# GradientSpaces/LivingScenes

Hardware: AMD Instinct MI355X
Metric: object-instances/sec (encode+match+register), N=1024 pts (higher is better)
Workload: dtype f32 (GEMM products as two-piece f16 splits on the f16 matrix cores, fp32 accumulate: as accurate against fp64 as an fp32 FMA chain)

## Files before the change

### livingscenes_amd/csrc/knn_common.h

```cpp
#pragma once
#include "ls_common.h"

namespace ls {

constexpr int KNN_TQ = 64;
constexpr int KNN_TS = 64;
constexpr int KNN_MAXK = 16;
constexpr int KNN_LD = KNN_TS + 4;

template <bool FMA>
__device__ __forceinline__ float accq(float d, float a, float b) {
#pragma clang fp contract(off)
    const float diff = a - b;
    if constexpr (FMA) {
        return __builtin_fmaf(diff, diff, d);
    } else {
        const float p = diff * diff;
        return d + p;
    }
}

typedef unsigned long long u64;
typedef float f32x2 __attribute__((ext_vector_type(2)));

template <bool FMA>
__device__ __forceinline__ f32x2 accq2(f32x2 d, float q, f32x2 c) {
#pragma clang fp contract(off)
    const f32x2 qq = {q, q};
    const f32x2 diff = qq - c;
    if constexpr (FMA) {
        return __builtin_elementwise_fma(diff, diff, d);
    } else {
        const f32x2 p = diff * diff;
        return d + p;
    }
}

__device__ __forceinline__ u64 make_key(float d, int idx, bool valid) {
    const u64 k = ((u64)__float_as_uint(d) << 32) | (unsigned)idx;
    return valid ? k : ~0ull;
}
__device__ __forceinline__ void key_cx(u64& a, u64& b) {
    const bool sw = b < a;
    const u64 lo = sw ? b : a, hi = sw ? a : b;
    a = lo; b = hi;
}
__device__ __forceinline__ u64 bperm64(int srclane, u64 v) {
    const unsigned lo = (unsigned)__builtin_amdgcn_ds_bpermute(srclane << 2, (int)(unsigned)v);
    const unsigned hi = (unsigned)__builtin_amdgcn_ds_bpermute(srclane << 2, (int)(unsigned)(v >> 32));
    return ((u64)hi << 32) | lo;
}
__device__ __forceinline__ u64 dpp_quad_bcast3(u64 v) {
    const unsigned lo = (unsigned)__builtin_amdgcn_update_dpp(0, (int)(unsigned)v, 0xFF, 0xF, 0xF, true);
    const unsigned hi = (unsigned)__builtin_amdgcn_update_dpp(0, (int)(unsigned)(v >> 32), 0xFF, 0xF, 0xF, true);
    return ((u64)hi << 32) | lo;
}
__device__ __forceinline__ u64 dpp_row_shr1(u64 v) {
    const unsigned lo = (unsigned)__builtin_amdgcn_update_dpp(0, (int)(unsigned)v, 0x111, 0xF, 0xF, false);
    const unsigned hi = (unsigned)__builtin_amdgcn_update_dpp(0, (int)(unsigned)(v >> 32), 0x111, 0xF, 0xF, false);
    return ((u64)hi << 32) | lo;
}

template <int CC>
struct Stager {
    static constexpr int U2 = CC / 16;
    static constexpr int PER = 3 * U2;
    float4 r[PER];
    __device__ __forceinline__ void load(const float* __restrict__ base, const int* rowmap, int row0, int nrows, size_t row_f,
                                         int C, int c0, int tid) {
        const int rr = tid >> 2, q = tid & 3;
        const int gr = rowmap ? rowmap[rr] : ((row0 + rr) < nrows ? row0 + rr : -1);
        const float* p = base + (size_t)(gr >= 0 ? gr : 0) * row_f + c0 + q * 4;
#pragma unroll
        for (int u = 0; u < PER; ++u) {
            const float4 v = *reinterpret_cast<const float4*>(p + (size_t)(u / U2) * C + (u % U2) * 16);
            r[u] = gr >= 0 ? v : make_float4(0.f, 0.f, 0.f, 0.f);
        }
    }
    __device__ __forceinline__ void store_pairs(float* lds, int PR, int tid) const {
        const int rr = tid >> 2, q = tid & 3;
        float* p0 = lds + (rr >> 1) * PR + (rr & 1) + 2 * (q * 12);
#pragma unroll
        for (int u = 0; u < PER; ++u) {
            float* p = p0 + 2 * ((u % U2) * 48 + (u / U2));
            p[0] = r[u].x; p[6] = r[u].y; p[12] = r[u].z; p[18] = r[u].w;
        }
    }
    __device__ __forceinline__ void store(float* lds, int ROW, int tid) const {
        const int rr = tid >> 2, q = tid & 3;
        float* p0 = lds + rr * ROW + q * 12;
#pragma unroll
        for (int u = 0; u < PER; ++u) {
            float* p = p0 + (u % U2) * 48 + (u / U2);
            p[0] = r[u].x; p[3] = r[u].y; p[6] = r[u].z; p[9] = r[u].w;
        }
    }
};


template <bool DEDUP>
__device__ __forceinline__ void merge_keys(u64 k0, u64 k1, u64 k2, u64 k3, u64& lkg, u64& kk, int K, int lane) {
    const int e16 = lane & 15, rowbase = lane & 48;
    u64 m64 = __ballot(k0 < kk);
    while (m64) {
        const unsigned rb = (unsigned)(m64 >> rowbase) & 0xFFFFu;
        bool rowhas = rb != 0;
        const int srclane = rowbase + __builtin_ctz(rb | 0x10000u);
        const u64 cand = bperm64(srclane, k0);
        const bool is_src = lane == srclane;
        k0 = is_src ? k1 : k0; k1 = is_src ? k2 : k1; k2 = is_src ? k3 : k2; k3 = is_src ? ~0ull : k3;
        if constexpr (DEDUP) {
            const u64 d64 = __ballot(rowhas & (lkg == cand));
            rowhas = rowhas & (((unsigned)(d64 >> rowbase) & 0xFFFFu) == 0u);
        }
        const u64 l64 = __ballot(rowhas & (lkg < cand));
        const int pos = __builtin_popcount((unsigned)(l64 >> rowbase) & 0xFFFFu);
        const u64 up = dpp_row_shr1(lkg);
        const bool s1 = rowhas & (e16 == pos), s2 = rowhas & (e16 > pos);
        lkg = s1 ? cand : (s2 ? up : lkg);
        kk = bperm64(rowbase + K - 1, lkg);
        m64 = __ballot(k0 < kk);
    }
}

template <bool DEDUP>
__device__ __forceinline__ void select_tile(const float* ldist, u64 (&lk)[4], u64 (&rkey)[4], int s0, int Ns, int K, int wave,
                                            int lane) {
    const int e16 = lane & 15;
#pragma unroll
    for (int g = 0; g < 4; ++g) {
        const int qrow = wave * 16 + g * 4 + (lane >> 4);
        const float4 dv = *reinterpret_cast<const float4*>(&ldist[qrow * KNN_LD + e16 * 4]);
        const int cbase = s0 + e16;
        u64 k0 = make_key(dv.x, cbase, cbase < Ns), k1 = make_key(dv.y, cbase + 16, cbase + 16 < Ns);
        u64 k2 = make_key(dv.z, cbase + 32, cbase + 32 < Ns), k3 = make_key(dv.w, cbase + 48, cbase + 48 < Ns);
        key_cx(k0, k1); key_cx(k2, k3); key_cx(k0, k2); key_cx(k1, k3); key_cx(k1, k2);
        merge_keys<DEDUP>(k0, k1, k2, k3, lk[g], rkey[g], K, lane);
    }
}

__device__ __forceinline__ void seed_lists(const u64* lseed, u64 (&lk)[4], u64 (&rkey)[4], int K, int wave, int lane) {
#pragma unroll
    for (int g = 0; g < 4; ++g) {
        const int qrow = wave * 16 + g * 4 + (lane >> 4);
        merge_keys<true>(lseed[qrow * 16 + (lane & 15)], ~0ull, ~0ull, ~0ull, lk[g], rkey[g], K, lane);
    }
}

template <bool FMA>
__device__ __forceinline__ float row_distance(const float* __restrict__ a, const float* __restrict__ b, int C) {
    float d = 0.0f;
    for (int c4 = 0; c4 < C; c4 += 4) {
        const float4 ax = *reinterpret_cast<const float4*>(a + c4), ay = *reinterpret_cast<const float4*>(a + C + c4),
                     az = *reinterpret_cast<const float4*>(a + 2 * C + c4);
        const float4 bx = *reinterpret_cast<const float4*>(b + c4), by = *reinterpret_cast<const float4*>(b + C + c4),
                     bz = *reinterpret_cast<const float4*>(b + 2 * C + c4);
        d = accq<FMA>(d, ax.x, bx.x); d = accq<FMA>(d, ay.x, by.x); d = accq<FMA>(d, az.x, bz.x);
        d = accq<FMA>(d, ax.y, bx.y); d = accq<FMA>(d, ay.y, by.y); d = accq<FMA>(d, az.y, bz.y);
        d = accq<FMA>(d, ax.z, bx.z); d = accq<FMA>(d, ay.z, by.z); d = accq<FMA>(d, az.z, bz.z);
        d = accq<FMA>(d, ax.w, bx.w); d = accq<FMA>(d, ay.w, by.w); d = accq<FMA>(d, az.w, bz.w);
    }
    return d;
}

template <bool FMA>
__device__ __forceinline__ void compute_seed_keys(u64* lseed, const int32_t* __restrict__ seed_idx, int seed_n, bool seed_by_row,
                                                  const float* __restrict__ dbase, const float* __restrict__ sbase, const int* lqrow,
                                                  int b, int q0, int Ns, int C, int tid) {
    const size_t row_f = (size_t)3 * C;
#pragma unroll
    for (int u = 0; u < 4; ++u) {
        const int p = tid + u * 256;
        const int q = p >> 4, e = p & 15;
        const int r = lqrow[q];
        int sidx = -1;
        if (r >= 0) sidx = seed_idx[((size_t)b * seed_n + (seed_by_row ? r : q0 + q)) * 16 + e];
        u64 key = ~0ull;
        if (sidx >= 0 && sidx < Ns) key = make_key(row_distance<FMA>(dbase + (size_t)r * row_f, sbase + (size_t)sidx * row_f, C), sidx, true);
        lseed[q * 16 + e] = key;
    }
}

__device__ __forceinline__ void write_lists(const u64 (&lk)[4], int b, int q0, int Nd, int K, int wave, int lane, int splits, int sp,
                                            u64* __restrict__ partial, int32_t* __restrict__ idx_out, float* __restrict__ dist_out) {
#pragma unroll
    for (int g = 0; g < 4; ++g) {
        const int q = q0 + wave * 16 + g * 4 + (lane >> 4);
        const int e = lane & 15;
        if (q < Nd && splits > 1) {
            partial[(((size_t)b * Nd + q) * splits + sp) * 16 + e] = e < K ? lk[g] : ~0ull;
        } else if (q < Nd && e < K) {
            const size_t o = ((size_t)b * Nd + q) * K + e;
            const unsigned hi = (unsigned)(lk[g] >> 32), lo = (unsigned)lk[g];
            idx_out[o] = hi == 0xFFFFFFFFu ? -1 : (int)lo;
            if (dist_out) dist_out[o] = hi == 0xFFFFFFFFu ? INFINITY : __uint_as_float(hi);
        }
    }
}

template <int CTRL>
__device__ __forceinline__ unsigned dpp_mov(unsigned v) {
    return (unsigned)__builtin_amdgcn_update_dpp(0, (int)v, CTRL, 0xF, 0xF, true);
}
template <int M>
__device__ __forceinline__ unsigned lane_xor(unsigned v, int lane) {
    if constexpr (M == 1) return dpp_mov<0xB1>(v);
    else if constexpr (M == 2) return dpp_mov<0x4E>(v);
    else if constexpr (M == 3) return dpp_mov<0x1B>(v);
    else if constexpr (M == 7) return dpp_mov<0x141>(v);
    else if constexpr (M == 15) return dpp_mov<0x140>(v);
    else if constexpr (M < 32) return (unsigned)__builtin_amdgcn_ds_swizzle((int)v, (M << 10) | 0x1F);
    else return (unsigned)__builtin_amdgcn_ds_bpermute((lane ^ M) << 2, (int)v);
}
template <int M>
__device__ __forceinline__ constexpr int pair_bit() { return (M & (M + 1)) == 0 ? (M + 1) / 2 : M; }

template <int M>
__device__ __forceinline__ void cx32(unsigned& v, int lane) {
    const unsigned o = lane_xor<M>(v, lane);
    v = (lane & pair_bit<M>()) == 0 ? min(v, o) : max(v, o);
}
template <int M>
__device__ __forceinline__ void cx64(u64& v, int lane) {
    const u64 o = ((u64)lane_xor<M>((unsigned)(v >> 32), lane) << 32) | lane_xor<M>((unsigned)v, lane);
    const bool lt = o < v, takemin = (lane & pair_bit<M>()) == 0;
    v = (takemin == lt) ? o : v;
}
__device__ __forceinline__ unsigned kth_smallest_upper_bound(unsigned v, int K) {
    unsigned ans = 0;
#pragma unroll
    for (int bit = 30; bit >= 15; --bit) {
        const unsigned t = ans | ((1u << bit) - 1u);
        const int cnt = __builtin_popcountll(__ballot(v <= t));
        ans |= cnt >= K ? 0u : (1u << bit);
    }
    return min(ans | 0x7FFFu, 0x7F800000u);
}

#define LS_SORT16(CX, v, lane)                                                                                         \
    CX<1>(v, lane);                                                                                                    \
    CX<3>(v, lane); CX<1>(v, lane);                                                                                    \
    CX<7>(v, lane); CX<2>(v, lane); CX<1>(v, lane);                                                                    \
    CX<15>(v, lane); CX<4>(v, lane); CX<2>(v, lane); CX<1>(v, lane);

#define LS_SORT32(CX, v, lane)                                                                                         \
    LS_SORT16(CX, v, lane)                                                                                             \
    CX<31>(v, lane); CX<8>(v, lane); CX<4>(v, lane); CX<2>(v, lane); CX<1>(v, lane);

#define LS_SORT64(CX, v, lane)                                                                                         \
    CX<1>(v, lane);                                                                                                    \
    CX<3>(v, lane); CX<1>(v, lane);                                                                                    \
    CX<7>(v, lane); CX<2>(v, lane); CX<1>(v, lane);                                                                    \
    CX<15>(v, lane); CX<4>(v, lane); CX<2>(v, lane); CX<1>(v, lane);                                                   \
    CX<31>(v, lane); CX<8>(v, lane); CX<4>(v, lane); CX<2>(v, lane); CX<1>(v, lane);                                   \
    CX<63>(v, lane); CX<16>(v, lane); CX<8>(v, lane); CX<4>(v, lane); CX<2>(v, lane); CX<1>(v, lane);


}
```

### livingscenes_amd/csrc/knn_mfma.hip

```cpp
#include "knn_common.h"

namespace ls {

typedef float f32x16 __attribute__((ext_vector_type(16)));


template <int CC>
struct QuadRow {
    float4 v[6];
    __device__ __forceinline__ void load(const float* __restrict__ row, int lane, int round = 0) {
        const int off = round * 32 + (lane & 3) * 8;
#pragma unroll
        for (int x = 0; x < 3; ++x)
#pragma unroll
            for (int h = 0; h < 2; ++h) v[x * 2 + h] = *reinterpret_cast<const float4*>(row + x * CC + off + 4 * h);
    }
};
template <int CC, bool FMA, bool LAST>
__device__ __forceinline__ float quad_round(float d, const QuadRow<CC>& q, const QuadRow<CC>& c) {
#pragma clang fp contract(off)
    float t[24];
#pragma unroll
    for (int h = 0; h < 2; ++h)
#pragma unroll
        for (int x = 0; x < 3; ++x) {
            const float4 a = q.v[x * 2 + h], b = c.v[x * 2 + h];
            const float d0 = a.x - b.x, d1 = a.y - b.y, d2 = a.z - b.z, d3 = a.w - b.w;
            t[(h * 4 + 0) * 3 + x] = FMA ? d0 : d0 * d0;
            t[(h * 4 + 1) * 3 + x] = FMA ? d1 : d1 * d1;
            t[(h * 4 + 2) * 3 + x] = FMA ? d2 : d2 * d2;
            t[(h * 4 + 3) * 3 + x] = FMA ? d3 : d3 * d3;
        }
#pragma unroll
    for (int s = 0; s < 4; ++s) {
#pragma unroll
        for (int j = 0; j < 24; ++j) d = FMA ? __builtin_fmaf(t[j], t[j], d) : d + t[j];
        if (s < 3)
            d = __int_as_float(__builtin_amdgcn_update_dpp(0, __float_as_int(d), 0x90, 0xF, 0xF, false));
        else if (!LAST)
            d = __int_as_float(__builtin_amdgcn_update_dpp(0, __float_as_int(d), 0x93, 0xF, 0xF, false));
    }
    return d;
}
template <int CC, bool FMA>
__device__ __forceinline__ float quad_pair_distance(const QuadRow<CC>& q0, const float* __restrict__ qrow, const float* __restrict__ crow,
                                                    int lane) {
    QuadRow<CC> c;
    c.load(crow, lane, 0);
    if constexpr (CC == 32) {
        return quad_round<CC, FMA, true>(0.0f, q0, c);
    } else {
        float d = quad_round<CC, FMA, false>(0.0f, q0, c);
#pragma unroll
        for (int r = 1; r < CC / 32; ++r) {
            QuadRow<CC> q;
            q.load(qrow, lane, r);
            c.load(crow, lane, r);
            d = (r == CC / 32 - 1) ? quad_round<CC, FMA, true>(d, q, c) : quad_round<CC, FMA, false>(d, q, c);
        }
        return d;
    }
}

typedef _Float16 f16x8k __attribute__((ext_vector_type(8)));
typedef _Float16 kh2_t __attribute__((ext_vector_type(2)));
typedef float kf2_t __attribute__((ext_vector_type(2)));
constexpr int KNN_CENTRE_ROWS = 16;
template <int KK, int WPT>
__global__ __launch_bounds__(64 * WPT) void knn_prep_f16_tile_kernel(const float* __restrict__ f, const float* __restrict__ fc, int Nc, int N, int Npad,
                                                                    unsigned short* __restrict__ out, float* __restrict__ norms, float* __restrict__ iscale,
                                                                    int32_t* __restrict__ zero_buf, long long zero_n) {
    constexpr int D = KK * 16, KPW = KK / WPT, DW = KPW * 16;
    static_assert(KK % WPT == 0 && DW <= 64, "a wave's dims fit one lane each for the centre");
    __shared__ __attribute__((aligned(16))) float lmu[WPT][64];
    __shared__ float lamax[WPT][32], lsum[WPT][32];
    for (long long i = (long long)blockIdx.x * (64 * WPT) + threadIdx.x; i < zero_n; i += (long long)gridDim.x * (64 * WPT)) zero_buf[i] = 0;
    const int lane = threadIdx.x & 63, w = __builtin_amdgcn_readfirstlane(threadIdx.x >> 6), j = lane & 31, h = lane >> 5;
    const int tpi = Npad >> 5, b = blockIdx.x / tpi, tile = blockIdx.x % tpi, r = tile * 32 + j;
    const bool live = r < N;
    const float* rp = f + ((size_t)b * N + (live ? r : 0)) * D + w * DW + h * 8;
    float4 x[KPW][2];
#pragma unroll
    for (int kk = 0; kk < KPW; ++kk) { x[kk][0] = *reinterpret_cast<const float4*>(rp + kk * 16); x[kk][1] = *reinterpret_cast<const float4*>(rp + kk * 16 + 4); }
    {
        const int nc = min(Nc, KNN_CENTRE_ROWS);
        const float* cp = fc + (size_t)b * Nc * D + w * DW + lane;
        if (lane < DW) {
            float s0 = 0.f, s1 = 0.f, s2 = 0.f, s3 = 0.f;
            for (int rr = 0; rr + 3 < nc; rr += 4) {
                s0 += cp[(size_t)rr * D]; s1 += cp[(size_t)(rr + 1) * D]; s2 += cp[(size_t)(rr + 2) * D]; s3 += cp[(size_t)(rr + 3) * D];
            }
            for (int rr = nc & ~3; rr < nc; ++rr) s0 += cp[(size_t)rr * D];
            lmu[w][lane] = ((s0 + s1) + (s2 + s3)) / (float)nc;
        }
        __builtin_amdgcn_s_waitcnt(0xc07f);
        __builtin_amdgcn_wave_barrier();
    }
    float c[KPW][8];
    float amax = 0.f;
#pragma unroll
    for (int kk = 0; kk < KPW; ++kk) {
        const float4 m0 = *reinterpret_cast<const float4*>(&lmu[w][kk * 16 + h * 8]), m1 = *reinterpret_cast<const float4*>(&lmu[w][kk * 16 + h * 8 + 4]);
        const float4 x0 = x[kk][0], x1 = x[kk][1];
        const float t[8] = {x0.x - m0.x, x0.y - m0.y, x0.z - m0.z, x0.w - m0.w, x1.x - m1.x, x1.y - m1.y, x1.z - m1.z, x1.w - m1.w};
#pragma unroll
        for (int i = 0; i < 8; ++i) { c[kk][i] = live ? t[i] : 0.f; amax = fmaxf(amax, fabsf(t[i])); }
    }
    amax = fmaxf(amax, __shfl_xor(amax, 32, 64));
    if (h == 0) lamax[w][j] = amax;
    __syncthreads();
#pragma unroll
    for (int u = 0; u < WPT; ++u) amax = fmaxf(amax, lamax[u][j]);
    unsigned be = (__float_as_uint(amax) >> 23) & 0xffu;
    be = be < 15u ? 15u : be;
    const float sc = live ? __uint_as_float((268u - be) << 23) : 0.f;
    unsigned short* op = out + ((((size_t)b * tpi + tile) * KK + w * KPW) * 64 + lane) * 8;
    float s = 0.f;
#pragma unroll
    for (int kk = 0; kk < KPW; ++kk) {
        unsigned pk[4];
#pragma unroll
        for (int i = 0; i < 4; ++i) {
            const float c0 = c[kk][2 * i], c1 = c[kk][2 * i + 1];
            s += c0 * c0 + c1 * c1;
            const kh2_t hv = __builtin_convertvector(kf2_t{c0 * sc, c1 * sc}, kh2_t);
            pk[i] = __builtin_bit_cast(unsigned, hv);
        }
        uint4 wv;
        wv.x = pk[0]; wv.y = pk[1]; wv.z = pk[2]; wv.w = pk[3];
        *reinterpret_cast<uint4*>(op + (size_t)kk * 512) = wv;
    }
    s += __shfl_xor(s, 32, 64);
    if (h == 0) lsum[w][j] = s;
    __syncthreads();
    if (w == 0 && h == 0 && live) {
        float t = lsum[0][j];
#pragma unroll
        for (int u = 1; u < WPT; ++u) t += lsum[u][j];
        norms[(size_t)b * N + r] = t;
        iscale[(size_t)b * N + r] = __uint_as_float((be - 14u) << 23);
    }
}
#ifndef LS_KF_PK
#define LS_KF_PK 1
#endif
constexpr int KF_QT = 32;
constexpr int KF_WAVES = 8;
constexpr int KF_LCAP = 64;
constexpr int KF_MAXNS = KF_WAVES * 4 * 32;

template <int CC>
struct KfLds {
    float qrows[KF_QT][3 * CC];
    float qnx[KF_QT], qny[KF_QT];
    unsigned hm[KF_QT][64];
    float T[KF_QT];
    int cnt[KF_QT];
    int base[KF_QT + 1];
    unsigned short list[KF_QT][KF_LCAP];
    unsigned plist[KF_QT * KF_LCAP];
    u64 keys[KF_QT][KF_LCAP];
};

template <int CC, bool FMA>
__device__ __noinline__ u64 kf_brute_row(const float* __restrict__ qrow, const float* __restrict__ sbase, int Ns, int lane) {
    constexpr int RF = 3 * CC;
    const int quad = lane >> 2;
    const bool qlast = (lane & 3) == 3;
    QuadRow<CC> qv;
    qv.load(qrow, lane);
    u64 best = ~0ull;
    for (int base = 0; base < Ns; base += 48) {
        u64 ks[3];
#pragma unroll
        for (int u = 0; u < 3; ++u) {
            const int c = base + u * 16 + quad;
            const bool v = c < Ns;
            ks[u] = make_key(quad_pair_distance<CC, FMA>(qv, qrow, sbase + (size_t)(v ? c : 0) * RF, lane), c, v & qlast);
        }
        const int src = ((lane & 15) << 2) + 3;
        const u64 n0 = bperm64(src, ks[0]), n1 = bperm64(src, ks[1]), n2 = bperm64(src, ks[2]);
        u64 k = lane < 16 ? best : (lane < 32 ? n0 : (lane < 48 ? n1 : n2));
        LS_SORT64(cx64, k, lane)
        best = k;
    }
    return best;
}

template <int CC, bool FMA, int TPW>
__global__ __launch_bounds__(64 * KF_WAVES, FMA ? 3 : 4) void knn_fused_kernel(const float* __restrict__ dstf, const float* __restrict__ srcf, const int32_t* __restrict__ dst_rows,
                                                                  const unsigned short* __restrict__ dq, const unsigned short* __restrict__ sq,
                                                                  const float* __restrict__ nrm_dst, const float* __restrict__ nrm_src,
                                                                  const float* __restrict__ isc_dst, const float* __restrict__ isc_src, int Nd, int dst_n,
                                                                  int dst_npad, int Ns, int ns_pad, int K, int qtiles, float eps,
                                                                  int32_t* __restrict__ idx_out, float* __restrict__ dist_out, int32_t* __restrict__ surv_cnt) {
    constexpr int D = 3 * CC, KK = D / 16, RF = 3 * CC;
    __shared__ __attribute__((aligned(16))) KfLds<CC> L;
    const int tid = threadIdx.x, lane = tid & 63;
    const int wave = __builtin_amdgcn_readfirstlane(tid >> 6);
    const int l31 = lane & 31, lh = lane >> 5;
    const int logical = xcd_remap(blockIdx.x, gridDim.x);
    const int b = logical / qtiles, q0 = (logical - b * qtiles) * KF_QT;
    const unsigned short* dqb = dq + (size_t)b * dst_npad * D;
    const unsigned short* sqb = sq + (size_t)b * ns_pad * D;
    const float* sbase = srcf + (size_t)b * Ns * RF;
    const float* dbase = dstf + (size_t)b * dst_n * RF;
    const int ntiles = ns_pad >> 5;

    for (int i = tid; i < KF_QT * (RF / 4); i += 64 * KF_WAVES) {
        const int qr = i / (RF / 4), c4 = i - qr * (RF / 4);
        const int q = min(q0 + qr, Nd - 1);
        const int r = dst_rows ? dst_rows[(size_t)b * Nd + q] : q;
        *reinterpret_cast<float4*>(&L.qrows[qr][c4 * 4]) = *reinterpret_cast<const float4*>(dbase + (size_t)r * RF + c4 * 4);
    }
    if (tid < KF_QT) {
        const int q = q0 + tid;
        const int r = q < Nd ? (dst_rows ? dst_rows[(size_t)b * Nd + q] : q) : 0;
        const float nq = nrm_dst[(size_t)b * dst_n + r], iq = isc_dst[(size_t)b * dst_n + r];
        L.qnx[tid] = q < Nd ? nq : 0.f;
        L.qny[tid] = q < Nd ? -2.0f * iq : 0.f;
        L.cnt[tid] = 0;
    }
    for (int i = tid; i < KF_QT * 64; i += 64 * KF_WAVES) (&L.hm[0][0])[i] = 0x7F800000u;

    f16x8k a[KK];
    {
        const int qi = q0 + l31;
        const int r = qi < Nd ? (dst_rows ? dst_rows[(size_t)b * Nd + qi] : qi) : 0;
        const unsigned short* ap = dqb + ((size_t)(r >> 5) * KK * 64 + lh * 32 + (r & 31)) * 8;
#pragma unroll
        for (int kk = 0; kk < KK; ++kk) a[kk] = __builtin_bit_cast(f16x8k, *reinterpret_cast<const uint4*>(ap + (size_t)kk * 512));
    }
    f32x16 S[TPW];
    float cns[TPW], cic[TPW];
    {
        f16x8k bf[2][KK];
        auto load_b = [&](int t, f16x8k (&dstb)[KK]) {
            const int tg = min(wave + KF_WAVES * t, ntiles - 1);
            const unsigned short* bp = sqb + ((size_t)tg * KK * 64 + lane) * 8;
#pragma unroll
            for (int kk = 0; kk < KK; ++kk) dstb[kk] = __builtin_bit_cast(f16x8k, *reinterpret_cast<const uint4*>(bp + (size_t)kk * 512));
        };
        load_b(0, bf[0]);
#pragma unroll
        for (int t = 0; t < TPW; ++t) {
            if (t + 1 < TPW) load_b(t + 1, bf[(t + 1) & 1]);
            const int cg = min((wave + KF_WAVES * t) * 32 + l31, Ns - 1);
            cns[t] = nrm_src[(size_t)b * Ns + cg];
            cic[t] = isc_src[(size_t)b * Ns + cg];
#pragma unroll
            for (int r = 0; r < 16; ++r) S[t][r] = 0.0f;
#pragma unroll
            for (int kk = 0; kk < KK; ++kk) S[t] = __builtin_amdgcn_mfma_f32_32x32x16_f16(a[kk], bf[t & 1][kk], S[t], 0, 0, 0);
        }
    }
    __syncthreads();
    bool colv[TPW];
#pragma unroll
    for (int t = 0; t < TPW; ++t) colv[t] = (wave + KF_WAVES * t) < ntiles && (wave + KF_WAVES * t) * 32 + l31 < Ns;
#if LS_KF_PK
    {
        const int slot = (wave & 1) * 32 + l31;
        kf2_t cn2[TPW], ci2[TPW];
#pragma unroll
        for (int t = 0; t < TPW; ++t) { const float cn = colv[t] ? cns[t] : INFINITY; cn2[t] = kf2_t{cn, cn}; ci2[t] = kf2_t{cic[t], cic[t]}; }
        const kf2_t eps2 = {eps, eps};
#pragma unroll
        for (int r = 0; r < 16; r += 2) {
            const int qr = (r & 3) + 8 * (r >> 2) + 4 * lh;
            const kf2_t qx = *reinterpret_cast<const kf2_t*>(&L.qnx[qr]), qy = *reinterpret_cast<const kf2_t*>(&L.qny[qr]);
            float hm0 = INFINITY, hm1 = INFINITY;
#pragma unroll
            for (int t = 0; t < TPW; ++t) {
                const kf2_t nn = qx + cn2[t], w = qy * ci2[t];
                const kf2_t sv = {S[t][r], S[t][r + 1]};
                const kf2_t dh = __builtin_elementwise_fma(sv, w, nn), e = eps2 * nn;
                const kf2_t hi = dh + e;
                kf2_t lo = dh - e;
                hm0 = fminf(hm0, hi.x); hm1 = fminf(hm1, hi.y);
                asm volatile("" : "+v"(lo));
                S[t][r] = lo.x; S[t][r + 1] = lo.y;
            }
            const float h0 = fmaxf(hm0, 0.0f), h1 = fmaxf(hm1, 0.0f);
            if (h0 < INFINITY) atomicMin(&L.hm[qr][slot], __float_as_uint(h0));
            if (h1 < INFINITY) atomicMin(&L.hm[qr + 1][slot], __float_as_uint(h1));
            if ((r & 3) == 2) __builtin_amdgcn_sched_barrier(0);
        }
    }
#else
    {
        const int slot = (wave & 1) * 32 + l31;
#pragma unroll
        for (int r = 0; r < 16; ++r) {
            const int qr = (r & 3) + 8 * (r >> 2) + 4 * lh;
            const float2 qn = make_float2(L.qnx[qr], L.qny[qr]);
            float hmin = INFINITY;
#pragma unroll
            for (int t = 0; t < TPW; ++t) {
                const float nn = qn.x + cns[t], w = qn.y * cic[t];
                const float dh = __builtin_fmaf(S[t][r], w, nn), e = eps * nn;
                hmin = colv[t] ? fminf(hmin, dh + e) : hmin;
                float lo = dh - e;
                asm volatile("" : "+v"(lo));
                S[t][r] = lo;
            }
            const float h = fmaxf(hmin, 0.0f);
            if (h < INFINITY) atomicMin(&L.hm[qr][slot], __float_as_uint(h));
            if ((r & 3) == 3) __builtin_amdgcn_sched_barrier(0);
        }
    }
#endif
    __syncthreads();
#pragma unroll
    for (int u = 0; u < KF_QT / KF_WAVES; ++u) {
        const int qr = wave * (KF_QT / KF_WAVES) + u;
        const unsigned tb = kth_smallest_upper_bound(L.hm[qr][lane], K < 64 ? K : 64);
        if (lane == 0) L.T[qr] = __uint_as_float(tb);
    }
    __syncthreads();
    {
        unsigned mask[TPW];
#pragma unroll
        for (int t = 0; t < TPW; ++t) mask[t] = 0;
#pragma unroll
        for (int r = 0; r < 16; ++r) {
            const float Tr = L.T[(r & 3) + 8 * (r >> 2) + 4 * lh];
#pragma unroll
            for (int t = 0; t < TPW; ++t) mask[t] |= (S[t][r] > Tr) ? 0u : (1u << r);
        }
#pragma unroll
        for (int t = 0; t < TPW; ++t) {
            const int cg = (wave + KF_WAVES * t) * 32 + l31;
            unsigned m = colv[t] ? mask[t] : 0u;
            while (m) {
                const int r = __builtin_ctz(m);
                m &= m - 1;
                const int qr = (r & 3) + 8 * (r >> 2) + 4 * lh;
                if (q0 + qr < Nd) {
                    const int pos = atomicAdd(&L.cnt[qr], 1);
                    if (pos < KF_LCAP) L.list[qr][pos] = (unsigned short)cg;
                }
            }
        }
    }
    __syncthreads();
    if (wave == 0) {
        const int c = (lane < KF_QT && L.cnt[lane] <= KF_LCAP) ? L.cnt[lane] : 0;
        int incl = c;
#pragma unroll
        for (int o = 1; o < KF_QT; o <<= 1) {
            const int v = __shfl_up(incl, o, 64);
            incl += lane >= o ? v : 0;
        }
        if (lane < KF_QT) L.base[lane] = incl - c;
        if (lane == KF_QT - 1) L.base[KF_QT] = incl;
        if (lane < KF_QT && q0 + lane < Nd && surv_cnt) surv_cnt[(size_t)b * Nd + q0 + lane] = -(L.cnt[lane] > KF_LCAP ? Ns : L.cnt[lane]) - 1;
    }
    __syncthreads();
    for (int i = tid; i < KF_QT * KF_LCAP; i += 64 * KF_WAVES) {
        const int qr = i / KF_LCAP, j = i - qr * KF_LCAP;
        const int c = L.cnt[qr];
        if (c <= KF_LCAP && j < c) L.plist[L.base[qr] + j] = (unsigned)L.list[qr][j] | ((unsigned)qr << 16) | ((unsigned)j << 21);
    }
    __syncthreads();
    {
        const int P = L.base[KF_QT];
        const int Q = wave * 16 + (lane >> 2);
        const bool qlast = (lane & 3) == 3;
        struct Pair { unsigned ent; bool v; QuadRow<CC> c; };
        auto fetch = [&](int p0, Pair& pr) {
            const int p = p0 + Q;
            pr.v = p < P;
            pr.ent = L.plist[pr.v ? p : 0];
            pr.c.load(sbase + (size_t)(pr.ent & 0xFFFFu) * RF, lane, 0);
        };
        auto finish = [&](const Pair& pr) {
            const int cand = pr.ent & 0xFFFFu, qr = (pr.ent >> 16) & 31, slot = pr.ent >> 21;
            const float* qrow = &L.qrows[qr][0];
            QuadRow<CC> qv;
            qv.load(qrow, lane);
            float d;
            if constexpr (CC == 32) {
                d = quad_round<CC, FMA, true>(0.0f, qv, pr.c);
            } else {
                const float* crow = sbase + (size_t)cand * RF;
                d = quad_round<CC, FMA, false>(0.0f, qv, pr.c);
#pragma unroll
                for (int r = 1; r < CC / 32; ++r) {
                    QuadRow<CC> q, c;
                    q.load(qrow, lane, r);
                    c.load(crow, lane, r);
                    d = (r == CC / 32 - 1) ? quad_round<CC, FMA, true>(d, q, c) : quad_round<CC, FMA, false>(d, q, c);
                }
            }
            if (pr.v && qlast) L.keys[qr][slot] = make_key(d, cand, true);
        };
        if (P > 0) {
            Pair pa, pb;
            fetch(0, pa);
            for (int p0 = 0; p0 < P; p0 += 2 * 16 * KF_WAVES) {
                fetch(p0 + 16 * KF_WAVES, pb);
                __builtin_amdgcn_sched_barrier(0);
                finish(pa);
                if (p0 + 16 * KF_WAVES < P) {
                    fetch(p0 + 2 * 16 * KF_WAVES, pa);
                    __builtin_amdgcn_sched_barrier(0);
                    finish(pb);
                }
            }
        }
    }
    __syncthreads();
    auto emit = [&](int qr, u64 k, int e) {
        const int q = q0 + qr;
        if (q < Nd && e < K) {
            const size_t o = ((size_t)b * Nd + q) * K + e;
            const unsigned hi = (unsigned)(k >> 32), lw = (unsigned)k;
            idx_out[o] = hi == 0xFFFFFFFFu ? -1 : (int)lw;
            if (dist_out) dist_out[o] = hi == 0xFFFFFFFFu ? INFINITY : __uint_as_float(hi);
        }
    };
#pragma unroll
    for (int u = 0; u < KF_QT / KF_WAVES; u += 2) {
        const int qa = wave * (KF_QT / KF_WAVES) + u, qb = qa + 1;
        const int ca = L.cnt[qa], cb = L.cnt[qb];
        if (ca <= 32 && cb <= 32) {
            const int qr = lh ? qb : qa, c = lh ? cb : ca;
            u64 k = l31 < c ? L.keys[qr][l31] : ~0ull;
            LS_SORT32(cx64, k, lane)
            emit(qr, k, l31);
        } else {
#pragma unroll
            for (int h = 0; h < 2; ++h) {
                const int qr = h ? qb : qa, c = h ? cb : ca;
                u64 k;
                if (c <= KF_LCAP) {
                    k = lane < c ? L.keys[qr][lane] : ~0ull;
                    LS_SORT64(cx64, k, lane)
                } else {
                    k = q0 + qr < Nd ? kf_brute_row<CC, FMA>(&L.qrows[qr][0], sbase, Ns, lane) : ~0ull;
                }
                emit(qr, k, lane);
            }
        }
    }
}

static inline size_t pad32(size_t n) { return (n + 31) & ~(size_t)31; }
static int knn_prep_launch(const float* f, const float* fc, int Nc, int B, int N, int Npad, int D, unsigned short* out, float* norms, float* iscale, hipStream_t st) {
    const int tiles = B * (Npad / 32);
    if (D == 96)
        hipLaunchKernelGGL((knn_prep_f16_tile_kernel<6, 3>), dim3(tiles), dim3(192), 0, st, f, fc, Nc, N, Npad, out, norms, iscale, (int32_t*)nullptr, 0LL);
    else
        hipLaunchKernelGGL((knn_prep_f16_tile_kernel<12, 4>), dim3(tiles), dim3(256), 0, st, f, fc, Nc, N, Npad, out, norms, iscale, (int32_t*)nullptr, 0LL);
    LS_LAUNCH_CHECK();
    return LS_OK;
}
int knn_sweep_max_ns() { return KF_MAXNS; }

struct KfScratch { float *nsrc, *ndst, *isrc, *idst; int32_t* cnt; unsigned short *sq, *dq; size_t bytes; };
static KfScratch kf_layout(void* scratch, int B, int Nd, int dst_n, int Ns, int D, bool self) {
    char* sc = (char*)scratch;
    size_t off = 0;
    auto take = [&](size_t bytes) { char* p = sc + off; off = (off + bytes + 255) & ~(size_t)255; return p; };
    KfScratch k;
    k.cnt = (int32_t*)take((size_t)B * Nd * sizeof(int32_t));
    k.nsrc = (float*)take((size_t)B * Ns * sizeof(float));
    k.ndst = self ? k.nsrc : (float*)take((size_t)B * dst_n * sizeof(float));
    k.isrc = (float*)take((size_t)B * Ns * sizeof(float));
    k.idst = self ? k.isrc : (float*)take((size_t)B * dst_n * sizeof(float));
    k.sq = (unsigned short*)take((size_t)B * pad32(Ns) * D * sizeof(unsigned short));
    k.dq = self ? k.sq : (unsigned short*)take((size_t)B * pad32(dst_n) * D * sizeof(unsigned short));
    k.bytes = off;
    return k;
}
size_t knn_sweep_scratch_bytes(int B, int Nd, int dst_n, int Ns, int C) { return kf_layout(nullptr, B, Nd, dst_n, Ns, 3 * C, false).bytes; }

template <int CC>
static int knn_sweep_launch_t(const float* dst, const float* src, const int32_t* dst_rows, int B, int Nd, int dst_n, int Ns, int K, bool fma,
                              int32_t* idx_out, float* dist_out, void* scratch, hipStream_t st) {
    constexpr int D = 3 * CC;
    const KfScratch k = kf_layout(scratch, B, Nd, dst_n, Ns, D, dst == src);
    const int ns_pad = (int)pad32(Ns), dst_npad = (int)pad32(dst_n);
    int rc = knn_prep_launch(src, src, Ns, B, Ns, ns_pad, D, k.sq, k.nsrc, k.isrc, st);
    if (rc != LS_OK) return rc;
    if (dst != src) {
        rc = knn_prep_launch(dst, src, Ns, B, dst_n, dst_npad, D, k.dq, k.ndst, k.idst, st);
        if (rc != LS_OK) return rc;
    }
    const int qtiles = cdiv(Nd, KF_QT), tpw = cdiv(ns_pad / 32, KF_WAVES);
    const float epsF = 1.02f * 0.0009765625f + 6.0f * (float)(D + 4) * 5.9604645e-8f + 9.5367431640625e-7f + 4.76837158203125e-7f;
#define LS_KF(T) do { if (fma) hipLaunchKernelGGL((knn_fused_kernel<CC, true, T>), dim3(B * qtiles), dim3(64 * KF_WAVES), 0, st, dst, src, dst_rows, k.dq, k.sq, k.ndst, k.nsrc, k.idst, k.isrc, Nd, dst_n, dst_npad, Ns, ns_pad, K, qtiles, epsF, idx_out, dist_out, k.cnt); \
                   else hipLaunchKernelGGL((knn_fused_kernel<CC, false, T>), dim3(B * qtiles), dim3(64 * KF_WAVES), 0, st, dst, src, dst_rows, k.dq, k.sq, k.ndst, k.nsrc, k.idst, k.isrc, Nd, dst_n, dst_npad, Ns, ns_pad, K, qtiles, epsF, idx_out, dist_out, k.cnt); } while (0)
    if (tpw <= 1) LS_KF(1); else if (tpw == 2) LS_KF(2); else LS_KF(4);
#undef LS_KF
    LS_LAUNCH_CHECK();
    return LS_OK;
}

int knn_sweep_launch(const float* dst, const float* src, const int32_t* dst_rows, int B, int Nd, int dst_n, int Ns, int C, int K,
                     bool fma, int32_t* idx_out, float* dist_out, const int32_t* , int , int , void* scratch,
                     hipStream_t st) {
    LS_REQUIRE(C == 32 || C == 64, "knn_sweep: only C == 32 / 64 layers are supported (C=%d)", C);
    LS_REQUIRE((int)pad32(Ns) <= KF_MAXNS && K <= KNN_MAXK, "knn_sweep: Ns=%d K=%d beyond the fused kernel (Ns <= %d, K <= 16)", Ns, K, KF_MAXNS);
    if (C == 32) return knn_sweep_launch_t<32>(dst, src, dst_rows, B, Nd, dst_n, Ns, K, fma, idx_out, dist_out, scratch, st);
    return knn_sweep_launch_t<64>(dst, src, dst_rows, B, Nd, dst_n, Ns, K, fma, idx_out, dist_out, scratch, st);
}

__global__ __launch_bounds__(256) void knn_stats_kernel(const int32_t* __restrict__ surv_cnt, long long nq, unsigned long long* __restrict__ out) {
    unsigned long long s = 0;
    for (long long i = (long long)blockIdx.x * 256 + threadIdx.x; i < nq; i += (long long)gridDim.x * 256) {
        const int c = surv_cnt[i];
        s += (unsigned long long)(c < 0 ? -(c + 1) : 0);
    }
    for (int o = 32; o > 0; o >>= 1) s += __shfl_xor(s, o, 64);
    if ((threadIdx.x & 63) == 0) atomicAdd(&out[0], s);
    if (blockIdx.x == 0 && threadIdx.x == 0) atomicAdd(&out[1], (unsigned long long)nq);
}
int knn_sweep_stats_launch(const void* scratch, int B, int Nd, int dst_n, int Ns, unsigned long long* out, hipStream_t st) {
    const size_t nq = (size_t)B * Nd;
    (void)dst_n; (void)Ns;
    hipLaunchKernelGGL(knn_stats_kernel, dim3((unsigned)std::min<size_t>(cdiv((long long)nq, 256), 256)), dim3(256), 0, st, (const int32_t*)scratch, (long long)nq, out);
    LS_LAUNCH_CHECK();
    return LS_OK;
}

}
```

### livingscenes_amd/csrc/knn_xyz.hip

```cpp
#include "knn_common.h"

namespace ls {

constexpr int KX_CH = 1024;

template <bool FMA, bool SINGLE>
__global__ __launch_bounds__(256, 4) void knn_xyz_kernel(const float* __restrict__ dst, const float* __restrict__ src,
                                                      const int32_t* __restrict__ dst_rows, int Nd, int dst_n, int Ns, int K,
                                                      int32_t* __restrict__ idx_out, float* __restrict__ dist_out, int qpw,
                                                      int qblocks) {
    __shared__ u64 lsurv[4][KX_CH + 1];
    const int lane = threadIdx.x & 63;
    const int wave = __builtin_amdgcn_readfirstlane(threadIdx.x >> 6);
    const int logical = xcd_remap(blockIdx.x, gridDim.x);
    const int b = logical / qblocks, qb = logical % qblocks;
    const float* sb = src + (size_t)b * Ns * 3;
    const float* db = dst + (size_t)b * dst_n * 3;
    u64* ls = lsurv[wave];
    constexpr bool single = SINGLE;

    f32x2 cx[8], cy[8], cz[8];
    auto load_chunk = [&](int c0) {
#pragma unroll
        for (int j = 0; j < 8; ++j) {
            const int ca = c0 + lane + 64 * j, cb = ca + 512;
            const int la = min(ca, Ns - 1), lb = min(cb, Ns - 1);
            const float ax = sb[(size_t)la * 3 + 0], ay = sb[(size_t)la * 3 + 1], az = sb[(size_t)la * 3 + 2];
            const float bx = sb[(size_t)lb * 3 + 0], by = sb[(size_t)lb * 3 + 1], bz = sb[(size_t)lb * 3 + 2];
            cx[j] = f32x2{ca < Ns ? ax : INFINITY, cb < Ns ? bx : INFINITY};
            cy[j] = f32x2{ca < Ns ? ay : INFINITY, cb < Ns ? by : INFINITY};
            cz[j] = f32x2{ca < Ns ? az : INFINITY, cb < Ns ? bz : INFINITY};
        }
    };
    if (single) load_chunk(0);

    const int qbase = (qb * 4 + wave) * qpw;
    for (int qi = 0; qi < qpw; ++qi) {
        const int q = qbase + qi;
        if (q >= Nd) break;
        const int r = __builtin_amdgcn_readfirstlane(dst_rows ? dst_rows[(size_t)b * Nd + q] : q);
        const float qx = db[(size_t)r * 3 + 0], qy = db[(size_t)r * 3 + 1], qz = db[(size_t)r * 3 + 2];
        u64 best = ~0ull;
        for (int c0 = 0; c0 < Ns; c0 += KX_CH) {
            if (!single) load_chunk(c0);
            f32x2 d[8];
            unsigned mn = 0x7F800000u;
#pragma unroll
            for (int j = 0; j < 8; ++j) {
                f32x2 a = accq2<FMA>(f32x2{0.0f, 0.0f}, qx, cx[j]);
                a = accq2<FMA>(a, qy, cy[j]);
                a = accq2<FMA>(a, qz, cz[j]);
                d[j] = a;
                mn = min(mn, min(__float_as_uint(a.x), __float_as_uint(a.y)));
            }
            unsigned thr = kth_smallest_upper_bound(mn, K);
            thr = min(thr, (unsigned)__builtin_amdgcn_readlane((int)(unsigned)(best >> 32), K - 1));
            thr = min(thr, 0x7F7FFFFFu);
            int n = 0;
#pragma unroll
            for (int jj = 0; jj < 16; ++jj) {
                const int j = jj & 7;
                const float dv = jj < 8 ? d[j].x : d[j].y;
                const int c = c0 + lane + 64 * j + (jj < 8 ? 0 : 512);
                const bool pass = __float_as_uint(dv) <= thr;
                const u64 bal = __ballot(pass);
                const int pos = n + (int)__builtin_amdgcn_mbcnt_hi((unsigned)(bal >> 32), __builtin_amdgcn_mbcnt_lo((unsigned)bal, 0u));
                ls[pass ? pos : KX_CH] = make_key(dv, c, true);
                n += __builtin_popcountll(bal);
            }
            __builtin_amdgcn_wave_barrier();
            int pos = 0;
            if (c0 == 0) {
                u64 k = lane < n ? ls[lane] : ~0ull;
                if (n <= 32) { LS_SORT32(cx64, k, lane) }
                else { LS_SORT64(cx64, k, lane) }
                best = k;
                pos = 64;
            }
            for (; pos < n; pos += 48) {
                u64 k = best;
                if (lane >= 16) {
                    const int i = pos + lane - 16;
                    k = i < n ? ls[i] : ~0ull;
                }
                LS_SORT64(cx64, k, lane)
                best = k;
            }
            __builtin_amdgcn_wave_barrier();
        }
        if (lane < K) {
            const size_t o = ((size_t)b * Nd + q) * K + lane;
            const unsigned hi = (unsigned)(best >> 32), lo = (unsigned)best;
            idx_out[o] = hi == 0xFFFFFFFFu ? -1 : (int)lo;
            if (dist_out) dist_out[o] = hi == 0xFFFFFFFFu ? INFINITY : __uint_as_float(hi);
        }
    }
}

int knn_xyz_launch(const float* dst, const float* src, const int32_t* dst_rows, int B, int Nd, int dst_n, int Ns, int K, bool fma,
                   int32_t* idx_out, float* dist_out, hipStream_t st) {
    int qpw = 16;
    while (qpw > 1 && (long long)B * cdiv(Nd, 4 * qpw) < 1024) qpw >>= 1;
    const int qblocks = cdiv(Nd, 4 * qpw);
    const bool single = Ns <= KX_CH;
#define LS_KX(F, S) hipLaunchKernelGGL((knn_xyz_kernel<F, S>), dim3(B * qblocks), dim3(256), 0, st, dst, src, dst_rows, Nd, dst_n, Ns, K, \
                                       idx_out, dist_out, qpw, qblocks)
    if (fma) { if (single) LS_KX(true, true); else LS_KX(true, false); }
    else { if (single) LS_KX(false, true); else LS_KX(false, false); }
#undef LS_KX
    LS_LAUNCH_CHECK();
    return LS_OK;
}


__device__ __forceinline__ int cdiv_dev(int a, int b) { return (a + b - 1) / b; }
constexpr int KSM_Q = 8, KSM_S = 32, KSM_CCH = 128;
constexpr int KSM_ROW = 3 * KSM_CCH + 4;

template <bool FMA>
__global__ __launch_bounds__(256, 2) void knn_small_kernel(const float* __restrict__ dstf, const float* __restrict__ srcf,
                                                           const int32_t* __restrict__ dst_rows, int Nd, int dst_n, int Ns, int C, int K,
                                                           int32_t* __restrict__ idx_out, float* __restrict__ dist_out, int qblocks) {
    LS_LATENCY_CRITICAL();
    __shared__ __attribute__((aligned(16))) float lq[KSM_Q * KSM_ROW];
    __shared__ __attribute__((aligned(16))) float lc[KSM_S * KSM_ROW];
    __shared__ float ldist[KSM_Q][KSM_S + 1];
    __shared__ int lqrow[KSM_Q];
    const int tid = threadIdx.x, lane = tid & 63, wave = tid >> 6;
    const int logical = xcd_remap(blockIdx.x, gridDim.x);
    const int b = logical / qblocks, q0 = (logical % qblocks) * KSM_Q;
    const size_t row_f = (size_t)3 * C;
    const float* dbase = dstf + (size_t)b * dst_n * row_f;
    const float* sbase = srcf + (size_t)b * Ns * row_f;
    if (tid < KSM_Q) {
        const int q = q0 + tid;
        lqrow[tid] = q < Nd ? (dst_rows ? dst_rows[(size_t)b * Nd + q] : q) : -1;
    }
    __syncthreads();
    const int qi = tid >> 5, ci = tid & 31;
    u64 lk = ~0ull, rkey = ~0ull;
    const int nch = cdiv_dev(C, KSM_CCH);
    const int sr = tid >> 3, sc = (tid & 7) * 4;
#define KSM_PF_LIST(F) F(0, 0) F(0, 1) F(0, 2) F(0, 3) F(1, 0) F(1, 1) F(1, 2) F(1, 3) F(2, 0) F(2, 1) F(2, 2) F(2, 3)
#define KSM_PF_DECL(x, m) float4 pf_##x##_##m;
#define KSM_PF_LOAD(x, m) pf_##x##_##m = *reinterpret_cast<const float4*>(rp + (size_t)x * C + min(m * 32, cwp - 32));
#define KSM_PF_STORE(x, m) \
    if (sc + m * 32 < cw) *reinterpret_cast<float4*>(&lc[sr * KSM_ROW + x * KSM_CCH + sc + m * 32]) = pf_##x##_##m;
    KSM_PF_LIST(KSM_PF_DECL)
#define KSM_PREFETCH(S0, CH)                                                                                  \
    {                                                                                                         \
        const int c0p = (CH) * KSM_CCH, cwp = min(C - c0p, KSM_CCH);                                          \
        const float* rp = sbase + (size_t)min((S0) + sr, Ns - 1) * row_f + c0p + sc;                          \
        KSM_PF_LIST(KSM_PF_LOAD)        \
    }
    KSM_PREFETCH(0, 0)
    for (int s0 = 0; s0 < Ns; s0 += KSM_S) {
        float d = 0.0f;
        for (int ch = 0; ch < nch; ++ch) {
            const int c0 = ch * KSM_CCH, cw = min(C - c0, KSM_CCH);
            __syncthreads();
            if (nch > 1 || s0 == 0) {
                const int gr = lqrow[qi];
                for (int x = 0; x < 3; ++x)
                    for (int c4 = ci * 4; c4 < cw; c4 += 128)
                        *reinterpret_cast<float4*>(&lq[qi * KSM_ROW + x * KSM_CCH + c4]) =
                            gr >= 0 ? *reinterpret_cast<const float4*>(dbase + (size_t)gr * row_f + (size_t)x * C + c0 + c4)
                                    : make_float4(0.f, 0.f, 0.f, 0.f);
            }
            KSM_PF_LIST(KSM_PF_STORE)
            __syncthreads();
            {
                int nch2 = ch + 1, ns0 = s0;
                if (nch2 == nch) { nch2 = 0; ns0 = s0 + KSM_S; }
                KSM_PREFETCH(min(ns0, Ns - 1), nch2)
            }
            const float* qp = &lq[qi * KSM_ROW];
            const float* cp = &lc[ci * KSM_ROW];
#pragma unroll 2
            for (int c4 = 0; c4 < cw; c4 += 4) {
                const float4 ax = *reinterpret_cast<const float4*>(qp + c4), ay = *reinterpret_cast<const float4*>(qp + KSM_CCH + c4),
                             az = *reinterpret_cast<const float4*>(qp + 2 * KSM_CCH + c4);
                const float4 bx = *reinterpret_cast<const float4*>(cp + c4), by = *reinterpret_cast<const float4*>(cp + KSM_CCH + c4),
                             bz = *reinterpret_cast<const float4*>(cp + 2 * KSM_CCH + c4);
                d = accq<FMA>(d, ax.x, bx.x); d = accq<FMA>(d, ay.x, by.x); d = accq<FMA>(d, az.x, bz.x);
                d = accq<FMA>(d, ax.y, bx.y); d = accq<FMA>(d, ay.y, by.y); d = accq<FMA>(d, az.y, bz.y);
                d = accq<FMA>(d, ax.z, bx.z); d = accq<FMA>(d, ay.z, by.z); d = accq<FMA>(d, az.z, bz.z);
                d = accq<FMA>(d, ax.w, bx.w); d = accq<FMA>(d, ay.w, by.w); d = accq<FMA>(d, az.w, bz.w);
            }
        }
        ldist[qi][ci] = d;
        __syncthreads();
        if (wave < 2) {
            const int qr = wave * 4 + (lane >> 4), e = lane & 15;
            const int ca = s0 + e, cb = s0 + e + 16;
            const bool live = lqrow[qr] >= 0;
            u64 k0 = make_key(ldist[qr][e], ca, live && ca < Ns), k1 = make_key(ldist[qr][e + 16], cb, live && cb < Ns);
            key_cx(k0, k1);
            merge_keys<false>(k0, k1, ~0ull, ~0ull, lk, rkey, K, lane);
        }
    }
    if (wave < 2) {
        const int qr = wave * 4 + (lane >> 4), e = lane & 15, q = q0 + qr;
        if (q < Nd && e < K) {
            const size_t o = ((size_t)b * Nd + q) * K + e;
            const unsigned hi = (unsigned)(lk >> 32), lo = (unsigned)lk;
            idx_out[o] = hi == 0xFFFFFFFFu ? -1 : (int)lo;
            if (dist_out) dist_out[o] = hi == 0xFFFFFFFFu ? INFINITY : __uint_as_float(hi);
        }
    }
}

int knn_small_launch(const float* dst, const float* src, const int32_t* dst_rows, int B, int Nd, int dst_n, int Ns, int C, int K, bool fma,
                     int32_t* idx_out, float* dist_out, hipStream_t st) {
    LS_REQUIRE(C % 4 == 0, "knn_small: C=%d must be a multiple of 4", C);
    const int qblocks = cdiv(Nd, KSM_Q);
    if (fma)
        hipLaunchKernelGGL(knn_small_kernel<true>, dim3(B * qblocks), dim3(256), 0, st, dst, src, dst_rows, Nd, dst_n, Ns, C, K, idx_out,
                           dist_out, qblocks);
    else
        hipLaunchKernelGGL(knn_small_kernel<false>, dim3(B * qblocks), dim3(256), 0, st, dst, src, dst_rows, Nd, dst_n, Ns, C, K, idx_out,
                           dist_out, qblocks);
    LS_LAUNCH_CHECK();
    return LS_OK;
}

}
```

Before: 57110.

## Compact KNN survivor lists with wave scans and overlap query staging with MFMA

The fused KNN filter kernel now builds its flat survivor pair list directly. A per-wave DPP inclusive scan and one atomic per wave replace the per-query list, the block-wide prefix pass and two extra barriers. Slot assignment into the per-query key buffers moves into the refine fetch step. Query-row staging into LDS is deferred until after the MFMA distance products, so its global loads can overlap the matrix work. The xyz kernel skips stores when a ballot is empty, and its launch heuristic targets more blocks. This adds a flood fallback when the shared pair list overflows, and registers rise from holding staged rows.

```diff
diff --git a/livingscenes_amd/csrc/knn_common.h b/livingscenes_amd/csrc/knn_common.h
--- a/livingscenes_amd/csrc/knn_common.h
+++ b/livingscenes_amd/csrc/knn_common.h
@@ -59,6 +59,16 @@
     const unsigned lo = (unsigned)__builtin_amdgcn_update_dpp(0, (int)(unsigned)v, 0x111, 0xF, 0xF, false);
     const unsigned hi = (unsigned)__builtin_amdgcn_update_dpp(0, (int)(unsigned)(v >> 32), 0x111, 0xF, 0xF, false);
     return ((u64)hi << 32) | lo;
+}
+
+__device__ __forceinline__ int wave_incl_scan(int v) {
+    v += __builtin_amdgcn_update_dpp(0, v, 0x111, 0xF, 0xF, false);
+    v += __builtin_amdgcn_update_dpp(0, v, 0x112, 0xF, 0xF, false);
+    v += __builtin_amdgcn_update_dpp(0, v, 0x114, 0xF, 0xF, false);
+    v += __builtin_amdgcn_update_dpp(0, v, 0x118, 0xF, 0xF, false);
+    v += __builtin_amdgcn_update_dpp(0, v, 0x142, 0xA, 0xF, false);
+    v += __builtin_amdgcn_update_dpp(0, v, 0x143, 0xC, 0xF, false);
+    return v;
 }
 
 template <int CC>
diff --git a/livingscenes_amd/csrc/knn_mfma.hip b/livingscenes_amd/csrc/knn_mfma.hip
--- a/livingscenes_amd/csrc/knn_mfma.hip
+++ b/livingscenes_amd/csrc/knn_mfma.hip
@@ -148,6 +148,7 @@
 constexpr int KF_WAVES = 8;
 constexpr int KF_LCAP = 64;
 constexpr int KF_MAXNS = KF_WAVES * 4 * 32;
+constexpr int KF_PCAP = KF_QT * KF_LCAP;
 
 template <int CC>
 struct KfLds {
@@ -156,9 +157,9 @@
     unsigned hm[KF_QT][64];
     float T[KF_QT];
     int cnt[KF_QT];
-    int base[KF_QT + 1];
-    unsigned short list[KF_QT][KF_LCAP];
-    unsigned plist[KF_QT * KF_LCAP];
+    int fill[KF_QT];
+    int np;
+    unsigned plist[KF_PCAP];
     u64 keys[KF_QT][KF_LCAP];
 };
 
@@ -207,22 +208,6 @@
     const float* dbase = dstf + (size_t)b * dst_n * RF;
     const int ntiles = ns_pad >> 5;
 
-    for (int i = tid; i < KF_QT * (RF / 4); i += 64 * KF_WAVES) {
-        const int qr = i / (RF / 4), c4 = i - qr * (RF / 4);
-        const int q = min(q0 + qr, Nd - 1);
-        const int r = dst_rows ? dst_rows[(size_t)b * Nd + q] : q;
-        *reinterpret_cast<float4*>(&L.qrows[qr][c4 * 4]) = *reinterpret_cast<const float4*>(dbase + (size_t)r * RF + c4 * 4);
-    }
-    if (tid < KF_QT) {
-        const int q = q0 + tid;
-        const int r = q < Nd ? (dst_rows ? dst_rows[(size_t)b * Nd + q] : q) : 0;
-        const float nq = nrm_dst[(size_t)b * dst_n + r], iq = isc_dst[(size_t)b * dst_n + r];
-        L.qnx[tid] = q < Nd ? nq : 0.f;
-        L.qny[tid] = q < Nd ? -2.0f * iq : 0.f;
-        L.cnt[tid] = 0;
-    }
-    for (int i = tid; i < KF_QT * 64; i += 64 * KF_WAVES) (&L.hm[0][0])[i] = 0x7F800000u;
-
     f16x8k a[KK];
     {
         const int qi = q0 + l31;
@@ -252,6 +237,34 @@
             for (int r = 0; r < 16; ++r) S[t][r] = 0.0f;
 #pragma unroll
             for (int kk = 0; kk < KK; ++kk) S[t] = __builtin_amdgcn_mfma_f32_32x32x16_f16(a[kk], bf[t & 1][kk], S[t], 0, 0, 0);
+        }
+    }
+    {
+        constexpr int NV = KF_QT * (RF / 4), TRIPS = (NV + 64 * KF_WAVES - 1) / (64 * KF_WAVES);
+        float4 rowv[TRIPS];
+#pragma unroll
+        for (int u = 0; u < TRIPS; ++u) {
+            const int i = min(tid + u * 64 * KF_WAVES, NV - 1);
+            const int qr = i / (RF / 4), c4 = i - qr * (RF / 4);
+            const int q = min(q0 + qr, Nd - 1);
+            const int r = dst_rows ? dst_rows[(size_t)b * Nd + q] : q;
+            rowv[u] = *reinterpret_cast<const float4*>(dbase + (size_t)r * RF + c4 * 4);
+        }
+        if (tid < KF_QT) {
+            const int q = q0 + tid;
+            const int r = q < Nd ? (dst_rows ? dst_rows[(size_t)b * Nd + q] : q) : 0;
+            const float nq = nrm_dst[(size_t)b * dst_n + r], iq = isc_dst[(size_t)b * dst_n + r];
+            L.qnx[tid] = q < Nd ? nq : 0.f;
+            L.qny[tid] = q < Nd ? -2.0f * iq : 0.f;
+            L.cnt[tid] = 0;
+            L.fill[tid] = 0;
+            if (tid == 0) L.np = 0;
+        }
+        for (int i = tid; i < KF_QT * 64; i += 64 * KF_WAVES) (&L.hm[0][0])[i] = 0x7F800000u;
+#pragma unroll
+        for (int u = 0; u < TRIPS; ++u) {
+            const int i = tid + u * 64 * KF_WAVES;
+            if (i < NV) *reinterpret_cast<float4*>(&(&L.qrows[0][0])[i * 4]) = rowv[u];
         }
     }
     __syncthreads();
@@ -319,6 +332,12 @@
     }
     __syncthreads();
     {
+        unsigned rowok = 0xFFFFu;
+        if (Nd - q0 < KF_QT) {
+            rowok = 0;
+#pragma unroll
+            for (int r = 0; r < 16; ++r) rowok |= q0 + (r & 3) + 8 * (r >> 2) + 4 * lh < Nd ? 1u << r : 0u;
+        }
         unsigned mask[TPW];
 #pragma unroll
         for (int t = 0; t < TPW; ++t) mask[t] = 0;
@@ -328,54 +347,50 @@
 #pragma unroll
             for (int t = 0; t < TPW; ++t) mask[t] |= (S[t][r] > Tr) ? 0u : (1u << r);
         }
+        int mine = 0;
 #pragma unroll
         for (int t = 0; t < TPW; ++t) {
-            const int cg = (wave + KF_WAVES * t) * 32 + l31;
-            unsigned m = colv[t] ? mask[t] : 0u;
+            mask[t] = colv[t] ? mask[t] & rowok : 0u;
+            mine += __builtin_popcount(mask[t]);
+        }
+        const int incl = wave_incl_scan(mine);
+        int wbase = 0;
+        if (lane == 63 && incl > 0) wbase = atomicAdd(&L.np, incl);
+        int pos = __builtin_amdgcn_readlane(wbase, 63) + incl - mine;
+#pragma unroll
+        for (int t = 0; t < TPW; ++t) {
+            const unsigned cg = (unsigned)((wave + KF_WAVES * t) * 32 + l31);
+            unsigned m = mask[t];
             while (m) {
                 const int r = __builtin_ctz(m);
                 m &= m - 1;
                 const int qr = (r & 3) + 8 * (r >> 2) + 4 * lh;
-                if (q0 + qr < Nd) {
-                    const int pos = atomicAdd(&L.cnt[qr], 1);
-                    if (pos < KF_LCAP) L.list[qr][pos] = (unsigned short)cg;
-                }
-            }
-        }
-    }
-    __syncthreads();
-    if (wave == 0) {
-        const int c = (lane < KF_QT && L.cnt[lane] <= KF_LCAP) ? L.cnt[lane] : 0;
-        int incl = c;
-#pragma unroll
-        for (int o = 1; o < KF_QT; o <<= 1) {
-            const int v = __shfl_up(incl, o, 64);
-            incl += lane >= o ? v : 0;
-        }
-        if (lane < KF_QT) L.base[lane] = incl - c;
-        if (lane == KF_QT - 1) L.base[KF_QT] = incl;
-        if (lane < KF_QT && q0 + lane < Nd && surv_cnt) surv_cnt[(size_t)b * Nd + q0 + lane] = -(L.cnt[lane] > KF_LCAP ? Ns : L.cnt[lane]) - 1;
-    }
-    __syncthreads();
-    for (int i = tid; i < KF_QT * KF_LCAP; i += 64 * KF_WAVES) {
-        const int qr = i / KF_LCAP, j = i - qr * KF_LCAP;
-        const int c = L.cnt[qr];
-        if (c <= KF_LCAP && j < c) L.plist[L.base[qr] + j] = (unsigned)L.list[qr][j] | ((unsigned)qr << 16) | ((unsigned)j << 21);
-    }
-    __syncthreads();
-    {
-        const int P = L.base[KF_QT];
+                atomicAdd(&L.cnt[qr], 1);
+                if (pos < KF_PCAP) L.plist[pos] = cg | ((unsigned)qr << 16);
+                ++pos;
+            }
+        }
+    }
+    __syncthreads();
+    const int np = L.np;
+    const bool flood = np > KF_PCAP;
+    if (tid < KF_QT && q0 + tid < Nd && surv_cnt)
+        surv_cnt[(size_t)b * Nd + q0 + tid] = -((flood || L.cnt[tid] > KF_LCAP) ? Ns : L.cnt[tid]) - 1;
+    {
+        const int P = flood ? 0 : np;
         const int Q = wave * 16 + (lane >> 2);
         const bool qlast = (lane & 3) == 3;
-        struct Pair { unsigned ent; bool v; QuadRow<CC> c; };
+        struct Pair { unsigned ent; int slot; QuadRow<CC> c; };
         auto fetch = [&](int p0, Pair& pr) {
             const int p = p0 + Q;
-            pr.v = p < P;
-            pr.ent = L.plist[pr.v ? p : 0];
+            const bool v = p < P;
+            pr.ent = L.plist[v ? p : 0];
+            pr.slot = KF_LCAP;
+            if (v && qlast) pr.slot = atomicAdd(&L.fill[pr.ent >> 16], 1);
             pr.c.load(sbase + (size_t)(pr.ent & 0xFFFFu) * RF, lane, 0);
         };
         auto finish = [&](const Pair& pr) {
-            const int cand = pr.ent & 0xFFFFu, qr = (pr.ent >> 16) & 31, slot = pr.ent >> 21;
+            const int cand = pr.ent & 0xFFFFu, qr = pr.ent >> 16;
             const float* qrow = &L.qrows[qr][0];
             QuadRow<CC> qv;
             qv.load(qrow, lane);
@@ -393,7 +408,7 @@
                     d = (r == CC / 32 - 1) ? quad_round<CC, FMA, true>(d, q, c) : quad_round<CC, FMA, false>(d, q, c);
                 }
             }
-            if (pr.v && qlast) L.keys[qr][slot] = make_key(d, cand, true);
+            if (pr.slot < KF_LCAP) L.keys[qr][pr.slot] = make_key(d, cand, true);
         };
         if (P > 0) {
             Pair pa, pb;
@@ -423,7 +438,7 @@
 #pragma unroll
     for (int u = 0; u < KF_QT / KF_WAVES; u += 2) {
         const int qa = wave * (KF_QT / KF_WAVES) + u, qb = qa + 1;
-        const int ca = L.cnt[qa], cb = L.cnt[qb];
+        const int ca = flood ? KF_LCAP + 1 : L.cnt[qa], cb = flood ? KF_LCAP + 1 : L.cnt[qb];
         if (ca <= 32 && cb <= 32) {
             const int qr = lh ? qb : qa, c = lh ? cb : ca;
             u64 k = l31 < c ? L.keys[qr][l31] : ~0ull;
diff --git a/livingscenes_amd/csrc/knn_xyz.hip b/livingscenes_amd/csrc/knn_xyz.hip
--- a/livingscenes_amd/csrc/knn_xyz.hip
+++ b/livingscenes_amd/csrc/knn_xyz.hip
@@ -9,7 +9,7 @@
                                                       const int32_t* __restrict__ dst_rows, int Nd, int dst_n, int Ns, int K,
                                                       int32_t* __restrict__ idx_out, float* __restrict__ dist_out, int qpw,
                                                       int qblocks) {
-    __shared__ u64 lsurv[4][KX_CH + 1];
+    __shared__ u64 lsurv[4][KX_CH];
     const int lane = threadIdx.x & 63;
     const int wave = __builtin_amdgcn_readfirstlane(threadIdx.x >> 6);
     const int logical = xcd_remap(blockIdx.x, gridDim.x);
@@ -61,12 +61,15 @@
             for (int jj = 0; jj < 16; ++jj) {
                 const int j = jj & 7;
                 const float dv = jj < 8 ? d[j].x : d[j].y;
-                const int c = c0 + lane + 64 * j + (jj < 8 ? 0 : 512);
                 const bool pass = __float_as_uint(dv) <= thr;
                 const u64 bal = __ballot(pass);
-                const int pos = n + (int)__builtin_amdgcn_mbcnt_hi((unsigned)(bal >> 32), __builtin_amdgcn_mbcnt_lo((unsigned)bal, 0u));
-                ls[pass ? pos : KX_CH] = make_key(dv, c, true);
-                n += __builtin_popcountll(bal);
+                if (bal) {
+                    if (pass) {
+                        const int pos = (int)__builtin_amdgcn_mbcnt_hi((unsigned)(bal >> 32), __builtin_amdgcn_mbcnt_lo((unsigned)bal, (unsigned)n));
+                        ls[pos] = make_key(dv, c0 + lane + 64 * j + (jj < 8 ? 0 : 512), true);
+                    }
+                    n += __builtin_popcountll(bal);
+                }
             }
             __builtin_amdgcn_wave_barrier();
             int pos = 0;
@@ -100,7 +103,7 @@
 int knn_xyz_launch(const float* dst, const float* src, const int32_t* dst_rows, int B, int Nd, int dst_n, int Ns, int K, bool fma,
                    int32_t* idx_out, float* dist_out, hipStream_t st) {
     int qpw = 16;
-    while (qpw > 1 && (long long)B * cdiv(Nd, 4 * qpw) < 1024) qpw >>= 1;
+    while (qpw > 1 && (long long)B * cdiv(Nd, 4 * qpw) < 2048) qpw >>= 1;
     const int qblocks = cdiv(Nd, 4 * qpw);
     const bool single = Ns <= KX_CH;
 #define LS_KX(F, S) hipLaunchKernelGGL((knn_xyz_kernel<F, S>), dim3(B * qblocks), dim3(256), 0, st, dst, src, dst_rows, Nd, dst_n, Ns, K, \
```

New measurement: 57450 (median of 6 runs). About the same (+0.6%).
